# MarioPasc/MGA-YOLO

Hardware: AMD Instinct MI355X
Metric: images/s (MaskCBAM fwd+bwd step at P3/P4/P5, YOLOv8n 640x640) (higher is better)
Workload: dtype f32; 1 GPU; YOLOv8n+MGA-CBAM P3/P4/P5, 32x640x640 synthetic per GPU, fp32 (BASELINE.json configs[1]); batch_per_gpu=32, global_batch=32, parallelism=dp1, launch=hipGraph replay, 1 graph/step, handoff_kernels=True

## Files before the change

### mga_yolo_amd/_lib.py

```python
from __future__ import annotations

import ctypes as C
import os
import threading
from typing import NamedTuple

_PKG = os.path.dirname(os.path.abspath(__file__))
LIB_PATH = os.environ.get("MGACBAM_LIB") or os.path.join(_PKG, "libmgacbam.so")
ABI_VERSION = 15
MAX_LEVELS = 8
F32, F16, BF16 = 0, 1, 2
E_NULL, E_SHAPE, E_DTYPE, E_ALIGN, E_LEVELS, E_SIZE = -1, -2, -3, -4, -5, -6
E_ARG = -7
FWD_STAGES = dict(pool=1, chan=2, apply=4)
BWD_STAGES = dict(reduce1=1, convT=2, reduce2=4, wsa=8, params=16, apply=32)
BWD_FUSE = 64
FWD_SAVE_PROJ, BWD_HAVE_PROJ, PROJ_MAX_HIDDEN = 1, 1, 4
LAYOUT_NHWC = 2
FWD_ALL, BWD_PARAMS, BWD_INPUTS, BWD_ALL = 7, 31, 32, 127
BWD_FOLD = 128
FWD_FUSE = 8

_c_float_p = C.POINTER(C.c_float)

# ... 446 lines not shown
    return nbytes


def seg_ws_bytes(levels, n: int) -> int:
    return _table_size("mgaseg_ws_bytes", E_SHAPE, levels, n)


def targets_scratch_bytes(desc) -> int:
    return _table_size("mgatgt_scratch_bytes", E_ARG, C.byref(desc), zero_is_an_answer=True)


def det_ws_bytes(desc) -> int:
    return _table_size("mgadet_ws_bytes", E_ARG, C.byref(desc))


def nms_ws_bytes(desc) -> int:
    return _table_size("mganms_ws_bytes", E_ARG, C.byref(desc))


def match_ws_bytes(desc) -> int:
    return _table_size("mgamatch_ws_bytes", E_ARG, C.byref(desc))


def sync_regions(B, Cc, H, W) -> dict:
    nf = B * ((H * W + 15) // 16 + 1)
    out, o = {}, 0
    for name, n in (("gate", nf), ("status", 4), ("ca", B), ("tiles", nf), ("conv_tiles", nf), ("merged_tiles", nf),
                    ("merged_conv_tiles", nf), ("wsa_tiles", nf), ("sweeps", B * Cc)):
        out[name] = (o, n)
        o += n
    return out


def sync_len(B, Cc, H, W) -> int:
    o, n = sync_regions(B, Cc, H, W)["sweeps"]
    return o + n


def sync_slices(B, Cc, H, W) -> dict:
    return {name: slice(o, o + n) for name, (o, n) in sync_regions(B, Cc, H, W).items()}


def ctx_layout(B, Cc, H, W, hidden) -> dict:
    key = ("layout", B, Cc, H, W, hidden)
    lay = _size_cache.get(key)
    if lay is None:
        L = CtxLayout()
        check(load().mgacbam_ctx_layout(B, Cc, H, W, hidden, C.byref(L)), "mgacbam_ctx_layout")
        lay = _size_cache[key] = {n: getattr(L, n) for n in CTX_FIELDS}
    return dict(lay)
```

### mga_yolo_amd/csrc/api_fwd.hip

```cpp
#include "host.cuh"
#include "fwd.cuh"
#include "nhwc_fwd.cuh"

struct FwdSig {
  int dtype, vec, has_mask, k, proj, gvec, nhwc, weight;
  bool operator==(const FwdSig& o) const {
    return dtype == o.dtype && vec == o.vec && has_mask == o.has_mask && k == o.k && proj == o.proj && gvec == o.gvec && nhwc == o.nhwc;
  }
};
static int forward_args(const mgacbam_fwd_level_t& L, FwdArgs& A, FwdSig& sig) {
  const bool nhwc = (L.flags & MGACBAM_LAYOUT_NHWC) != 0;
  if (!L.x || !L.y || !L.ctx || (nhwc && !L.ws))
    return fail(MGACBAM_E_NULL, nhwc ? "forward (NHWC): x / y / ctx / ws is NULL" : "forward: x / y / ctx is NULL");
  if (int e = check_level("forward", L)) return e;
  const int VEC = level_vec(nhwc, L.C, L.H, L.W, L.dtype);
  const size_t need = VEC * elem_size(L.dtype);
  if (!aligned_to(L.x, need) || !aligned_to(L.y, need) || !aligned_to(L.ctx, 16) || (nhwc && !aligned_to(L.ws, 16)) ||
      (L.mask && !aligned_to(L.mask, nhwc ? 4 : 16)))
    return fail(MGACBAM_E_ALIGN, "forward%s: x/y must be %zu-byte aligned, ctx%s 16-byte, mask %d-byte", nhwc ? " (NHWC)" : "", need,
                nhwc ? " / ws" : "", nhwc ? 4 : VEC * 4);
  if (int e = check_ctx_capacity("forward", L)) return e;
  if (nhwc) if (int e = check_capacity("forward", "ws", nhwc_ws_bytes(L.B, L.C, L.H, L.W, VEC), L.ws_bytes)) return e;
  A.x = L.x; A.mask = L.mask; A.y = L.y; A.fused = 0;
  level_setup(L, A);
  A.fault = knobs().fault;
  A.n = NhwcGeo{}; A.ws = nullptr;
  sig = FwdSig{};
  sig.dtype = L.dtype; sig.vec = VEC; sig.has_mask = L.mask != nullptr; sig.k = L.p.k; sig.nhwc = nhwc;
  if (nhwc) {
    A.n = nhwc_geo(L.C, L.H, L.W, VEC);
    A.ws = static_cast<float*>(L.ws);
    const int rows = std::min((A.n.ch - 1) / L.W + 2, L.H);
    A.t.apply_rows = rows + L.p.k - 1;
    sig.weight = L.C;
    return 0;
  }
  sig.weight = L.C * A.t.chan_tx;
  sig.proj = (L.flags & MGACBAM_FWD_SAVE_PROJ) && L.mask != nullptr;
  A.g.proj_h = (sig.proj && L.p.hidden <= MGACBAM_PROJ_MAX_HIDDEN) ? L.p.hidden : 0;
  sig.gvec = VEC;
  if (L.dtype != MGACBAM_F32 && VEC == 4 && (static_cast<long long>(L.H) * L.W) % 8 == 0) {
    Tune t8 = A.t;
    gate_geometry(L.C, L.H, L.W, L.p.k, 8, t8);
    if (t8.gate_tx > 0) { sig.gvec = 8; A.t = t8; }
  }
  return 0;
}

static int launch_mlp(Group<FwdArgs>& G, hipStream_t st) {
  return launch_group("k_mlp", k_mlp, G, [](const FwdArgs& a) { return a.g.B; }, [](const FwdArgs& a) { return mlp_smem(a.g); }, st);
}

static int forward_group_nhwc(FwdArgs* lv, int n, const FwdSig& sig, int stages, hipStream_t st);
static int forward_group(FwdArgs* lv, int n, const FwdSig& sig, int stages, hipStream_t st) {
  if (sig.nhwc) return forward_group_nhwc(lv, n, sig, stages, st);
  const int pool_cpt = group_cpt(lv, n);
  for (int l = 0; l < n; ++l) lv[l].t.pool_cpt = pool_cpt;
  Group<FwdArgs> G = make_group(lv, n);

  const int gvec = sig.gvec;
  bool gate = (stages & MGACBAM_FWD_FUSE) && (stages & MGACBAM_FWD_CHAN) && (stages & MGACBAM_FWD_APPLY) && !sig.proj && gvec > 0;
  for (int l = 0; l < n && gate; ++l) gate = lv[l].t.gate_tx > 0;
  void (*gate_kernel)(GateGroup) = nullptr;
  size_t gsmem = 0;
  if (gate) {
    int span = 0;
    for (int l = 0; l < n; ++l) span = std::max(span, lv[l].t.gate_span);
    gsmem = group_smem(G, [&](const FwdArgs& a) { return gate_smem(a.g, a.t, gvec); });
    gate_kernel = with_elem_vec8(sig.dtype, gvec, [&](auto t, auto v) {
      return with_k7(sig.k, [&](auto k) { return k_gate<elem_t<decltype(t)>, v.value, k.value>; }); });
    gate = 2 * (8 * span + 1) <= resident_workgroups(gate_kernel, gsmem);
  }
  if (gate) for (int l = 0; l < n; ++l) { lv[l].fused = 1; G.lv[l].fused = 1; }

  if (stages & MGACBAM_FWD_POOL) {
    auto kernel = with_elem_vec(sig.dtype, sig.vec, [&](auto t, auto v) { return with_cpt(pool_cpt, [&](auto c) {
      return with_bool(sig.has_mask, [&](auto m) { return k_pool<elem_t<decltype(t)>, v.value, c.value, m.value>; }); }); });
    if (int e = launch_group("k_pool", kernel, G, [&](const FwdArgs& a) { return sweep_blocks(a, a.t.pool_tx, pool_cpt); }, 0, st)) return e;
  }
  if (gate) {
    GateGroup GG;
    const int tiles = fill_starts(G, lv, n, [&](const FwdArgs& a) { return xcd_grid(a.g.B, gate_tiles(a.t, a.g.H, a.g.W, gvec)); });
    GG.g = G;
    GG.nrole = 0;
    for (int l = 0; l < n; ++l) { GG.rstart[l] = GG.nrole; GG.nrole += lv[l].g.B; }
    GG.rstart[n] = GG.nrole;
    return launch("k_gate", gate_kernel, GG.nrole + tiles, kBlock, gsmem, st, GG);
  }
  if (stages & MGACBAM_FWD_CHAN) {
    bool split_mlp = false;
    for (int l = 0; l < n; ++l) split_mlp |= static_cast<long long>(lv[l].g.C) * lv[l].g.hidden >= 8192;
    if (split_mlp) if (int e = launch_mlp(G, st)) return e;
    auto kernel = with_elem_vec(sig.dtype, sig.vec, [&](auto t, auto v) { return with_bool(sig.proj, [&](auto pj) {
      return with_bool(split_mlp, [&](auto sp) { return k_chan<elem_t<decltype(t)>, v.value, pj.value, sp.value>; }); }); });
    if (int e = launch_group("k_chan", kernel, G, [&](const FwdArgs& a) { return xcd_grid(a.g.B, chan_tiles(a.t, a.g.H, a.g.W, sig.vec)); },
                             [&](const FwdArgs& a) { return chan_smem(a.g, sig.vec, sig.proj); }, st)) return e;
  }
  if (stages & MGACBAM_FWD_APPLY) {
    auto kernel = with_elem_vec(sig.dtype, sig.vec, [&](auto t, auto v) {
      return with_k(sig.k, [&](auto k) { return k_apply<elem_t<decltype(t)>, v.value, k.value>; }); });
    if (int e = launch_group("k_apply", kernel, G, [&](const FwdArgs& a) { return xcd_grid(a.g.B, chan_tiles(a.t, a.g.H, a.g.W, sig.vec)); },
                             [&](const FwdArgs& a) { return apply_smem(a.g, a.t, sig.vec); }, st)) return e;
  }
  return 0;
}

static int forward_group_nhwc(FwdArgs* lv, int n, const FwdSig& sig, int stages, hipStream_t st) {
  Group<FwdArgs> G = make_group(lv, n);
  if (stages & MGACBAM_FWD_POOL) {
    auto pool = with_elem_vec8(sig.dtype, sig.vec, [&](auto t, auto v) {
      return with_bool(sig.has_mask, [&](auto m) { return k_pool_nhwc<elem_t<decltype(t)>, v.value, m.value>; }); });
    if (int e = launch_group("k_pool_nhwc", pool, G, [](const FwdArgs& a) { return xcd_grid(a.g.B, a.n.nchunk); },
                             [](const FwdArgs& a) { return nhwc_pool_smem(a.g); }, st)) return e;
    auto fin = with_bool(sig.has_mask, [](auto m) { return k_pool_fin<m.value>; });
    if (int e = launch_group("k_pool_fin", fin, G, [](const FwdArgs& a) { return nhwc_fold_blocks(a.g); }, 0, st)) return e;
    if (int e = launch_mlp(G, st)) return e;
  }
// ... 23 lines not shown
```

### mga_yolo_amd/csrc/args.cuh

```cuda
#pragma once
#include <stddef.h>
#include <stdint.h>

namespace mgacbam {

struct Geo {
  int B, C, H, W, HW;
  int hidden, k;
  int use_sigmoid;
  float thr, eps;
  int proj_h;
};
constexpr int kProjMax = 4;
constexpr int kProjWide = 16;
constexpr int kGateR = 16;
constexpr int kSyncPx = 16;

struct CtxPtrs {
  float* S; float* use; float* den;
  float* avg; float* mx; float* mavg;
  int* valid; int* amax;
  float* h_avg; float* h_mx; float* ca;
  float* planes; int* cidx; float* sa;
  float* proj;
  int* sync;
};

struct ParamPtrs { const float* w1; const float* b1; const float* w2; const float* b2; const float* wsa; const float* beta; };

struct Tune {
  int pool_tx;
  int pool_cpt;
  int chan_tx;
  int conv_twq;
  int conv_th;
  int wsa_th;
  int apply_rows;
  int gate_rows;
  int gate_tx;
  int gate_span;
};

struct NhwcGeo {
  int cs, lcs;
  int ng;
  int ch;
  int ntile;
  int rp;
  int nchunk;
};
constexpr int kNhwcMaxChunks = 64;
constexpr int kNhwcFoldC = 64;

struct FwdArgs {
  const void* x; const float* mask; void* y;
  CtxPtrs c; ParamPtrs p; Geo g; Tune t;
  int nflag;
  int fused;
  unsigned spin_limit;
  int fault;
  long long* trace;
  NhwcGeo n;
  float* ws;
};

struct ScratchPtrs {
  float* A_part;
  float* gpre;
  float* gplanes;
  float* gwsa_part;
  float* gz;
  float* gbq;
  float* gh_avg;
  float* gh_mx;
  float* pgh;
  float* proj;
};

struct BwdArgs {
  const void* x; const float* mask; const void* gy; void* gx; float* gmask;
  float* gw1; float* gb1; float* gw2; float* gb2; float* gwsa; float* gbeta;
  CtxPtrs c; ParamPtrs p; ScratchPtrs s; Geo g; Tune t;
  int nt;
  int nconv;
// ... 32 lines not shown
```

### mga_yolo_amd/csrc/common.cuh

```cuda
#pragma once
#include <hip/hip_runtime.h>
#include <hip/hip_fp16.h>
#include <hip/hip_bf16.h>
#include <float.h>
#include <stdint.h>

#include "args.cuh"

namespace mgacbam {

constexpr int kBlock = 256;
constexpr int kSweepPF = 1;
constexpr int kWave = 64;
using bf16_t = __hip_bfloat16;

template <typename T> __device__ __forceinline__ float to_f32(T v);
template <> __device__ __forceinline__ float to_f32<float>(float v) { return v; }
template <> __device__ __forceinline__ float to_f32<__half>(__half v) { return __half2float(v); }
template <> __device__ __forceinline__ float to_f32<bf16_t>(bf16_t v) { return __bfloat162float(v); }

template <typename T> __device__ __forceinline__ T from_f32(float v);
template <> __device__ __forceinline__ float from_f32<float>(float v) { return v; }
template <> __device__ __forceinline__ __half from_f32<__half>(float v) { return __float2half_rn(v); }
template <> __device__ __forceinline__ bf16_t from_f32<bf16_t>(float v) { return __float2bfloat16(v); }
// ... 149 lines not shown
    }
    __syncthreads();
    const int waves_per_row = TX >> 6;
    if ((tid & (TX - 1)) == 0) {
#pragma unroll
      for (int n = 0; n < N; ++n) {
        for (int w = 1; w < waves_per_row; ++w) argmax_combine(v[n], idx[n], red[(wave + w) * N + n], redi[(wave + w) * N + n]);
      }
    }
  }
}

__device__ __forceinline__ float block_sum(float v, int tid, float* red) {
  v = wave_group_sum(v, kWave);
  __syncthreads();
  if ((tid & 63) == 0) red[tid >> 6] = v;
  __syncthreads();
  if (tid == 0) { v = red[0]; for (int w = 1; w < kBlock / kWave; ++w) v += red[w]; }
  return v;
}

__device__ __forceinline__ int ilog2(int v) { return 31 - __clz(v); }

__device__ __forceinline__ void bilinear_tap(float scale, int d, int n, int& i0, int& i1, float& lam) {
  const float f = fmaxf(scale * (static_cast<float>(d) + 0.5f) - 0.5f, 0.f);
  i0 = min(static_cast<int>(f), n - 1);
  i1 = i0 + (i0 < n - 1 ? 1 : 0);
  lam = f - static_cast<float>(i0);
}

__device__ __forceinline__ bool xcd_sample_part(int bid, int B, int P, int& b, int& part) {
  const int x = bid & 7, q = bid >> 3;
  const int g8 = q / P;
  part = q - g8 * P;
  b = g8 * 8 + x;
  return b < B;
}

__device__ __forceinline__ float ld_agent(const float* p) { return __hip_atomic_load(p, __ATOMIC_RELAXED, __HIP_MEMORY_SCOPE_AGENT); }
__device__ __forceinline__ int ld_agent(const int* p) { return __hip_atomic_load(p, __ATOMIC_RELAXED, __HIP_MEMORY_SCOPE_AGENT); }
__device__ __forceinline__ void st_agent(float* p, float v) { __hip_atomic_store(p, v, __ATOMIC_RELAXED, __HIP_MEMORY_SCOPE_AGENT); }
__device__ __forceinline__ void st_agent(int* p, int v) { __hip_atomic_store(p, v, __ATOMIC_RELAXED, __HIP_MEMORY_SCOPE_AGENT); }
__device__ __forceinline__ void handoff_publish(int* flag) {
  asm volatile("s_waitcnt vmcnt(0)" ::: "memory");
  __syncthreads();
  if (threadIdx.x == 0) __hip_atomic_fetch_add(flag, 1, __ATOMIC_RELAXED, __HIP_MEMORY_SCOPE_AGENT);
// ... 52 lines not shown
```

### mga_yolo_amd/csrc/fwd.cuh

```cuda
#pragma once
#include "args.cuh"
#include "common.cuh"
#include "tile.cuh"

namespace mgacbam {

constexpr float kSelLogit = 0x1.8p-24f;

template <typename T, int VEC, int CPT, bool HAS_MASK>
__device__ __forceinline__ void pool_body(const FwdArgs& A, const int bid, float* red) {
  const Geo& g = A.g;
  const int tid = threadIdx.x;
  const int TX = A.t.pool_tx, lt = ilog2(TX);
  const int tx = tid & (TX - 1), ty = tid >> lt, TY = kBlock >> lt;
  const int CPB = TY * CPT;
  const int ncg = (g.C + CPB - 1) / CPB;
  int b, cg;
  if (!xcd_sample_part(bid, g.B, ncg, b, cg)) return;
  const int c0 = cg * CPB + ty * CPT;
  const int nv = g.HW / VEC;
  TRACE_HWID(A.trace, blockIdx.x);
  TRACE_MARK(A.trace, blockIdx.x, 0);

  const T* xr[CPT];
#pragma unroll
  for (int j = 0; j < CPT; ++j) {
    const int c = min(c0 + j, g.C - 1);
    xr[j] = static_cast<const T*>(A.x) + (static_cast<size_t>(b) * g.C + c) * g.HW;
  }
  const float* mb = HAS_MASK ? A.mask + static_cast<size_t>(b) * g.HW : nullptr;
  float* splane = A.c.planes + (static_cast<size_t>(b) * 3 + 2) * g.HW;
  const bool writes_plane = (cg == 0 && ty == 0);

  float sx[CPT], sxs[CPT], vmax[CPT];
  int imax[CPT];
#pragma unroll
  for (int j = 0; j < CPT; ++j) { sx[j] = 0.f; sxs[j] = 0.f; vmax[j] = -FLT_MAX; imax[j] = 0; }
  float ssum = 0.f;

  constexpr int PF = kSweepPF;
  for (int i0 = tx; i0 < nv; i0 += TX * PF) {
    float m[PF][VEC], xv[PF][CPT][VEC];
    bool ok[PF];
#pragma unroll
    for (int p = 0; p < PF; ++p) {
      const int i = i0 + p * TX;
      ok[p] = i < nv;
      const size_t o = static_cast<size_t>(ok[p] ? i : nv - 1) * VEC;
      if (HAS_MASK) load_vec<float, VEC>(mb + o, m[p]);
#pragma unroll
      for (int j = 0; j < CPT; ++j) load_vec<T, VEC>(xr[j] + o, xv[p][j]);
    }
#pragma unroll
    for (int p = 0; p < PF; ++p) {
      if (!ok[p]) continue;
// ... 34 lines not shown
  row_argmax<CPT>(vmax, imax, TX, tid, red);

  if (tx == 0) {
    const float N = static_cast<float>(g.HW);
    const float S = sums[2 * CPT];
    const float use = (S / N >= g.thr) ? 1.f : 0.f;
    const float den = fmaxf(S, g.eps);
#pragma unroll
    for (int j = 0; j < CPT; ++j) {
      const int c = c0 + j;
      if (c < g.C) {
        const size_t o = static_cast<size_t>(b) * g.C + c;
        const float gap = sums[j] / N;
        float avg, mavg, mxo;
        int valid;
        if (HAS_MASK) {
          mavg = sums[CPT + j] / den;
          avg = mavg * use + gap * (1.f - use);
          valid = isclosef_(vmax[j], -FLT_MAX) ? 0 : 1;
          mxo = valid ? vmax[j] : gap;
        } else {
          mavg = gap; avg = gap; valid = 1; mxo = vmax[j];
        }
        A.c.avg[o] = avg; A.c.mavg[o] = mavg; A.c.mx[o] = mxo;
        A.c.valid[o] = valid; A.c.amax[o] = imax[j];
      }
    }
    if (cg == 0 && ty == 0) {
      A.c.S[b] = HAS_MASK ? S : 0.f;
      A.c.use[b] = HAS_MASK ? use : 0.f;
      A.c.den[b] = HAS_MASK ? den : 1.f;
    }
  }
#ifdef MGACBAM_TRACE
  TRACE_MARK(A.trace, blockIdx.x, 8);
  asm volatile("s_waitcnt vmcnt(0)" ::: "memory");
  __syncthreads();
  TRACE_MARK(A.trace, blockIdx.x, 10);
#endif
}

template <typename T, int VEC, int CPT, bool HAS_MASK>
__global__ __launch_bounds__(kBlock) void k_pool(const Group<FwdArgs> G) {
  __shared__ float red[64];
  int local;
  const int l = find_level(G, blockIdx.x, local);
  pool_body<T, VEC, CPT, HAS_MASK>(G.lv[l], local, red);
}

__device__ __forceinline__ void mlp_gate_to_lds(const FwdArgs& A, const int b, const bool publish,
                                                float* s_in, float* s_h, float* s_ca) {
  const Geo& g = A.g;
  const int tid = threadIdx.x, C = g.C, h = g.hidden;
  const int wave = tid >> 6, lane = tid & 63;
  float* s_avg = s_in;
  float* s_mx = s_in + C;
  for (int c = tid; c < C; c += kBlock) {
    s_avg[c] = A.c.avg[static_cast<size_t>(b) * C + c];
    s_mx[c] = A.c.mx[static_cast<size_t>(b) * C + c];
  }
  __syncthreads();
  for (int j = wave; j < h; j += kBlock / kWave) {
    const float* w = A.p.w1 + static_cast<size_t>(j) * C;
    float da = 0.f, dm = 0.f;
    for (int c = lane; c < C; c += kWave) { const float wv = w[c]; da += wv * s_avg[c]; dm += wv * s_mx[c]; }
    da = wave_group_sum(da, kWave);
    dm = wave_group_sum(dm, kWave);
    if (lane == 0) {
      const float bj = A.p.b1[j];
      const float ha = fmaxf(da + bj, 0.f), hm = fmaxf(dm + bj, 0.f);
// ... 281 lines not shown
  const int nv = g.HW / VEC;
  const int ntile = (nv + TX - 1) / TX;
  int b, tile;
  if (!xcd_sample_part(bid, g.B, ntile, b, tile)) return;
  const int i = tile * TX + tx;
  const bool active = i < nv;
  const int ii = active ? i : nv - 1;
  const size_t base = static_cast<size_t>(b) * g.C * g.HW + static_cast<size_t>(ii) * VEC;
  const T* xp = static_cast<const T*>(A.x) + base;
  T* yp = static_cast<T*>(A.y) + base;

  const int gid = blockIdx.x;
  TRACE_HWID(A.trace, gid);
  TRACE_MARK(A.trace, gid, 0);
  Pack<T, VEC> xr[R];
#pragma unroll
  for (int j = 0; j < R; ++j)
    xr[j] = *reinterpret_cast<const Pack<T, VEC>*>(xp + static_cast<size_t>(min(ty + j * TY, g.C - 1)) * g.HW);
  int* flags = A.c.sync + static_cast<size_t>(b) * A.nflag;
  const int gen = static_cast<int>(static_cast<unsigned>(ld_agent(flags + tile)) + 1u);

  float* s_ca = smem;
  float* work = s_ca + ((g.C + 3) & ~3);
  bool bad;
  {
    int* caflag = A.c.sync + static_cast<size_t>(g.B) * A.nflag + 4;
    bad = handoff_wait(caflag, b, b, gen, caflag - 4, A.spin_limit);
    const float* cab = A.c.ca + static_cast<size_t>(b) * g.C;
    TRACE_MARK(A.trace, gid, 1);
    for (int c = tid; c < g.C; c += kBlock) s_ca[c] = ld_agent(cab + c);
    __syncthreads();
  }
  TRACE_MARK(A.trace, gid, 2);

  float vmax[VEC], vsum[VEC];
  int vidx[VEC];
#pragma unroll
  for (int e = 0; e < VEC; ++e) { vmax[e] = -INFINITY; vsum[e] = 0.f; vidx[e] = ty; }
#pragma unroll
  for (int j = 0; j < R; ++j) {
    const int c = ty + j * TY;
    if (c < g.C) {
      const float cac = s_ca[c];
#pragma unroll
      for (int e = 0; e < VEC; ++e) {
        const float uu = to_f32<T>(xr[j].v[e]) * cac;
        vsum[e] += uu;
        if (uu > vmax[e]) { vmax[e] = uu; vidx[e] = c; }
      }
    }
  }
  TRACE_MARK(A.trace, gid, 3);
  {
// ... 112 lines not shown
#pragma unroll
  for (int j = 0; j < R; ++j) {
    const int c = ty + j * TY;
    if (c < g.C) {
      const float cac = s_ca[c];
      float yv[VEC];
#pragma unroll
      for (int e = 0; e < VEC; ++e) {
        const float xe = to_f32<T>(xr[j].v[e]);
        const float u = xe * cac;
        yv[e] = xe + a * (u * sav[e] - xe);
      }
      if (active) store_vec<T, VEC>(yp + static_cast<size_t>(c) * g.HW, yv);
    }
  }
#ifdef MGACBAM_TRACE
  TRACE_MARK(A.trace, gid, 9);
  asm volatile("s_waitcnt vmcnt(0)" ::: "memory");
  __syncthreads();
  TRACE_MARK(A.trace, gid, 10);
#endif
}

constexpr int kMlpW1 = 8;
constexpr int kMlpW2 = 8;
__device__ __forceinline__ bool mlp_stream_ok(const Geo& g) { return (g.C & 3) == 0 && (g.hidden & 3) == 0 && g.C <= 8 * 4 * kWave; }

template <int CVL>
__device__ __forceinline__ void mlp_hidden(const FwdArgs& A, const int b, float* s_avg, float* s_mx, float* s_h) {
  constexpr int UP = kMlpW1 / CVL;
  const Geo& g = A.g;
  const int tid = threadIdx.x, C = g.C, h = g.hidden, CV = C >> 2;
  const int wave = tid >> 6, lane = tid & 63;
  const float4* w1v = reinterpret_cast<const float4*>(A.p.w1);
  const int nunit = h > wave ? (h - wave + 3) >> 2 : 0;
  const int npass = (((h + 3) >> 2) + UP - 1) / UP;
  for (int p = 0; p < npass; ++p) {
    float4 wr[UP][CVL];
#pragma unroll
    for (int uu = 0; uu < UP; ++uu) {
      const int u = p * UP + uu, j = wave + 4 * u;
#pragma unroll
      for (int i = 0; i < CVL; ++i) {
        const int cv = lane + kWave * i;
        wr[uu][i] = (u < nunit && cv < CV) ? w1v[static_cast<size_t>(j) * CV + cv] : float4{0.f, 0.f, 0.f, 0.f};
      }
    }
    if (p == 0) {
      for (int c = tid; c < C; c += kBlock) {
        s_avg[c] = A.c.avg[static_cast<size_t>(b) * C + c];
        s_mx[c] = A.c.mx[static_cast<size_t>(b) * C + c];
      }
      __syncthreads();
    }
#pragma unroll
    for (int uu = 0; uu < UP; ++uu) {
      const int u = p * UP + uu;
      if (u < nunit) {
        float da = 0.f, dm = 0.f;
#pragma unroll
        for (int i = 0; i < CVL; ++i) {
          const int cv = lane + kWave * i;
          if (cv < CV) {
            const float4 w = wr[uu][i];
            const float4 a4 = *reinterpret_cast<const float4*>(s_avg + 4 * cv), m4 = *reinterpret_cast<const float4*>(s_mx + 4 * cv);
            da += w.x * a4.x + w.y * a4.y + w.z * a4.z + w.w * a4.w;
            dm += w.x * m4.x + w.y * m4.y + w.z * m4.z + w.w * m4.w;
          }
        }
        da = wave_group_sum(da, kWave);
        dm = wave_group_sum(dm, kWave);
        if (lane == 0) {
          const int j = wave + 4 * u;
          const float bj = A.p.b1[j];
          const float ha = fmaxf(da + bj, 0.f), hm = fmaxf(dm + bj, 0.f);
          s_h[j] = ha; s_h[h + j] = hm;
          A.c.h_avg[static_cast<size_t>(b) * h + j] = ha;
          A.c.h_mx[static_cast<size_t>(b) * h + j] = hm;
        }
      }
    }
  }
}

template <bool AGENT>
__device__ __forceinline__ void mlp_stream(const FwdArgs& A, const int b, float* smem) {
  const Geo& g = A.g;
  const int tid = threadIdx.x, C = g.C, h = g.hidden;
  float* s_avg = smem;
  float* s_mx = smem + C;
  float* s_h = smem + 2 * C;
  const int cvl = ((C >> 2) + kWave - 1) / kWave;
  if (cvl <= 1) mlp_hidden<1>(A, b, s_avg, s_mx, s_h);
  else if (cvl <= 2) mlp_hidden<2>(A, b, s_avg, s_mx, s_h);
  else if (cvl <= 4) mlp_hidden<4>(A, b, s_avg, s_mx, s_h);
  else mlp_hidden<8>(A, b, s_avg, s_mx, s_h);
  const int HV = h >> 2;
  const float4* w2v = reinterpret_cast<const float4*>(A.p.w2);
  float4 wr[kMlpW2];
  {
    const int c = min(tid, C - 1);
#pragma unroll
    for (int q = 0; q < kMlpW2; ++q) wr[q] = q < HV ? w2v[static_cast<size_t>(c) * HV + q] : float4{0.f, 0.f, 0.f, 0.f};
  }
  __syncthreads();
  for (int c = tid; c < C; c += kBlock) {
    float za = 0.f, zm = 0.f;
    for (int v0 = 0; v0 < HV; v0 += kMlpW2) {
      if (c != tid || v0 != 0) {
#pragma unroll
        for (int q = 0; q < kMlpW2; ++q) wr[q] = v0 + q < HV ? w2v[static_cast<size_t>(c) * HV + v0 + q] : float4{0.f, 0.f, 0.f, 0.f};
      }
#pragma unroll
      for (int q = 0; q < kMlpW2; ++q) {
        if (v0 + q < HV) {
          const float* ha = s_h + 4 * (v0 + q);
          const float* hm = ha + h;
          za += wr[q].x * ha[0]; zm += wr[q].x * hm[0];
          za += wr[q].y * ha[1]; zm += wr[q].y * hm[1];
          za += wr[q].z * ha[2]; zm += wr[q].z * hm[2];
          za += wr[q].w * ha[3]; zm += wr[q].w * hm[3];
        }
      }
    }
    const float bc = A.p.b2[c];
    const float ca = sigmoidf_((za + bc) + (zm + bc));
    if (AGENT) st_agent(A.c.ca + static_cast<size_t>(b) * C + c, ca);
    else A.c.ca[static_cast<size_t>(b) * C + c] = ca;
  }
}

__device__ __forceinline__ void gate_role(const FwdArgs& A, const int b, float* smem) {
  const Geo& g = A.g;
  const int tid = threadIdx.x, C = g.C, h = g.hidden;
  int* caflag = A.c.sync + static_cast<size_t>(g.B) * A.nflag + 4 + b;
  TRACE_MARK(A.trace, blockIdx.x, 0);
  if (mlp_stream_ok(g)) {
// ... 58 lines not shown
```

### mga_yolo_amd/csrc/host.cuh

```cuda
#pragma once
#include "../../include/mgacbam.h"

#include <hip/hip_runtime.h>
#include <stdarg.h>
#include <stdio.h>
#include <stdlib.h>
#include <string.h>

#include <algorithm>
#include <atomic>
#include <map>
#include <mutex>
#include <type_traits>
#include <utility>

#include "args.cuh"
#include "common.cuh"

using namespace mgacbam;

inline thread_local char g_err[512] = "";
static int fail(int code, const char* fmt, ...) {
  va_list ap;
  va_start(ap, fmt);
// ... 7 lines not shown
  void* p[] = {const_cast<void*>(static_cast<const void*>(&args))...};
  const hipError_t e = hipLaunchKernel(reinterpret_cast<const void*>(kernel), dim3(static_cast<unsigned>(grid)), dim3(block), p, smem, st);
  if (e != hipSuccess) return fail(static_cast<int>(e), "%s: %s", what, hipGetErrorString(e));
  return 0;
}

static int check_shape(int B, int C, int H, int W, int hidden, int k) {
  if (B < 1 || C < 1 || H < 1 || W < 1 || hidden < 1 || hidden > 4096 || C > 65536)
    return fail(MGACBAM_E_SHAPE, "bad shape B=%d C=%d H=%d W=%d hidden=%d", B, C, H, W, hidden);
  if (static_cast<long long>(H) * W > (1ll << 30) || static_cast<long long>(B) * C * H * W > (1ll << 40))
    return fail(MGACBAM_E_SHAPE, "tensor too large B=%d C=%d H=%d W=%d", B, C, H, W);
  if (k < 1 || k > 15 || (k & 1) == 0) return fail(MGACBAM_E_SHAPE, "spatial kernel k=%d must be odd and in 1..15", k);
  return 0;
}

struct SyncLayout {
  size_t nflag;
  size_t gate;
  size_t status;
  size_t ca;
  size_t bflag, cflag;
  size_t mbflag, mcflag;
  size_t wflag, sflag;
  size_t len;
};
static SyncLayout sync_layout(int B, int C, size_t HW) {
  SyncLayout S;
  S.nflag = (HW + kSyncPx - 1) / kSyncPx + 1;
  const size_t per = static_cast<size_t>(B) * S.nflag;
  S.gate = 0; S.status = per; S.ca = S.status + 4; S.bflag = S.ca + B;
  S.cflag = S.bflag + per; S.mbflag = S.cflag + per; S.mcflag = S.mbflag + per; S.wflag = S.mcflag + per; S.sflag = S.wflag + per;
  S.len = S.sflag + static_cast<size_t>(B) * C;
  return S;
}

struct Carver {
  size_t total = 0;
  size_t take(size_t n_elems) { const size_t off = total; total = align16(total + n_elems * 4); return off; }
};
template <typename T = float>
static T* at(const void* base, size_t off) { return reinterpret_cast<T*>(static_cast<char*>(const_cast<void*>(base)) + off); }

static void ctx_layout(int B, int C, int H, int W, int hidden, mgacbam_ctx_layout_t* L) {
  const size_t HW = static_cast<size_t>(H) * W, BC = static_cast<size_t>(B) * C;
  Carver cv;
  L->S = cv.take(B); L->use = cv.take(B); L->den = cv.take(B);
  L->avg = cv.take(BC); L->mx = cv.take(BC); L->mavg = cv.take(BC);
  L->valid = cv.take(BC); L->amax = cv.take(BC);
  L->h_avg = cv.take(static_cast<size_t>(B) * hidden); L->h_mx = cv.take(static_cast<size_t>(B) * hidden);
  L->ca = cv.take(BC);
  L->planes = cv.take(static_cast<size_t>(B) * 3 * HW);
  L->cidx = cv.take(static_cast<size_t>(B) * HW);
  L->sa = cv.take(static_cast<size_t>(B) * HW);
  L->proj = cv.take(hidden <= MGACBAM_PROJ_MAX_HIDDEN ? static_cast<size_t>(B) * hidden * HW : 0);
  const SyncLayout S = sync_layout(B, C, HW);
// ... 1 lines not shown
  L->status = L->sync + static_cast<int64_t>(4 * S.status);
  L->total = static_cast<int64_t>(cv.total);
}

static CtxPtrs ctx_ptrs(void* p, int B, int C, int H, int W, int hidden) {
  mgacbam_ctx_layout_t L;
  ctx_layout(B, C, H, W, hidden, &L);
  return CtxPtrs{at(p, L.S), at(p, L.use), at(p, L.den), at(p, L.avg), at(p, L.mx), at(p, L.mavg), at<int>(p, L.valid), at<int>(p, L.amax),
                 at(p, L.h_avg), at(p, L.h_mx), at(p, L.ca), at(p, L.planes), at<int>(p, L.cidx), at(p, L.sa), at(p, L.proj), at<int>(p, L.sync)};
}

static int pow2_floor(int v) { int p = 1; while (p * 2 <= v) p *= 2; return p; }
static int pow2_ceil(int v) { int p = 1; while (p < v) p *= 2; return p; }
static int env_int(const char* name, int dflt) {
  const char* s = getenv(name);
  return (s && *s) ? atoi(s) : dflt;
}
struct Knobs {
  int bwd_merge;
  int gate_narrow;
  int pool_tx, pool_cpt, chan_tx;
  int resident_wgs;
  int fault;
  unsigned spin_limit;
  long long* trace;
};
static Knobs read_knobs() {
  Knobs k;
  k.bwd_merge = env_int("MGACBAM_BWD_MERGE", 1);
  k.gate_narrow = env_int("MGACBAM_GATE_NARROW", 0);
  k.pool_tx = env_int("MGACBAM_POOL_TX", 0); k.pool_cpt = env_int("MGACBAM_POOL_CPT", 0); k.chan_tx = env_int("MGACBAM_CHAN_TX", 0);
  k.resident_wgs = env_int("MGACBAM_RESIDENT_WGS", 0); k.fault = env_int("MGACBAM_FAULT", 0);
  const int sl = env_int("MGACBAM_SPIN_LIMIT", 0);
  k.spin_limit = sl > 0 ? static_cast<unsigned>(sl) : (1u << 20);
  const char* tp = getenv("MGACBAM_TRACE_PTR");
  k.trace = (tp && *tp) ? reinterpret_cast<long long*>(strtoull(tp, nullptr, 0)) : nullptr;
  return k;
}
inline std::mutex g_knob_mu;
inline Knobs g_knobs;
inline std::atomic<bool> g_knobs_ready{false};
static Knobs knobs() {
  if (!g_knobs_ready.load(std::memory_order_acquire)) {
    std::lock_guard<std::mutex> lk(g_knob_mu);
    if (!g_knobs_ready.load(std::memory_order_relaxed)) { g_knobs = read_knobs(); g_knobs_ready.store(true, std::memory_order_release); }
  }
  return g_knobs;
}

static int device_cus() {
  static std::mutex mu;
  static int cus[64] = {0};
  int dev = 0;
  if (hipGetDevice(&dev) != hipSuccess || dev < 0 || dev >= 64) return 0;
  std::lock_guard<std::mutex> lk(mu);
// ... 21 lines not shown
    int n = 0;
    if (hipOccupancyMaxActiveBlocksPerMultiprocessor(&n, kernel, kBlock, smem) != hipSuccess) n = 0;
    per_cu = n;
    std::lock_guard<std::mutex> lk(mu);
    cache[key] = per_cu;
  }
  return per_cu * device_cus();
}
static bool is_pow2_in(int v, int lo, int hi) { return v >= lo && v <= hi && (v & (v - 1)) == 0; }

static int vec_of(int H, int W) { return (static_cast<long long>(H) * W) % 4 == 0 ? 4 : 1; }

static void gate_geometry(int C, int H, int W, int k, int VEC, Tune& t) {
  t.gate_tx = 0; t.gate_rows = 0; t.gate_span = 0;
  const int gty = pow2_ceil((C + kGateR - 1) / kGateR);
  if (gty > kBlock) return;
  const int gtx = kBlock / gty, TP = gtx * VEC;
  int grows = (TP - 1) / W + 2;
  if (grows > H) grows = H;
  grows += k - 1;
  const int span = ((k / 2) * W + TP - 1) / TP + 1;
  const size_t lds = (3 * static_cast<size_t>(grows) * (W + k - 1) + TP + 3 * k * k + 3 * C + 64) * sizeof(float);
  if (TP >= kSyncPx && (TP >= W || knobs().gate_narrow) && lds <= 48 * 1024) { t.gate_tx = gtx; t.gate_rows = grows; t.gate_span = span; }
}

static Tune choose_tune(int B, int C, int H, int W, int k) {
  const int HW = H * W, VEC = vec_of(H, W), nv = HW / VEC;
  const Knobs kn = knobs();
  Tune t;
  int tx = pow2_floor(nv / 4 > 0 ? nv / 4 : 1);
  if (tx > 256) tx = 256;
  int cpt = 4;
  while (cpt > 1 && static_cast<long long>(B) * ((C + (256 / tx) * cpt - 1) / ((256 / tx) * cpt)) < 1024) cpt /= 2;
  t.pool_tx = tx; t.pool_cpt = cpt;
  int ctx = pow2_ceil(nv) < 64 ? pow2_ceil(nv) : 64;
  constexpr int kChanMinTx = 16;
  while (ctx > kChanMinTx && static_cast<long long>(B) * ((nv + ctx - 1) / ctx) < 768) ctx /= 2;
  while (ctx < 64 && (256 / ctx) * 4 > C) ctx *= 2;
  t.chan_tx = ctx;
  const int ntx = (W + 127) / 128;
  const int tw = (((W + ntx - 1) / ntx) + 3) / 4 * 4;
  t.conv_twq = tw / 4;
  int th = 256 / t.conv_twq;
  if (th > H) th = H;
  if (th > 64) th = 64;
  const int cap = 24 * 256 / (4 * (tw + k - 1)) - (k - 1);
// ... 202 lines not shown
static int params_blocks(const Geo& g) { return g.hidden + (g.C + kBlock - 1) / kBlock + (3 * g.k * g.k + 3) / 4 + 1; }
static size_t chan_smem(const Geo& g, int vec, bool proj) {
  return (3 * static_cast<size_t>(g.C) + 2 * g.hidden + (proj ? static_cast<size_t>(g.C) * kProjMax : 0) + 4 * kBlock * vec) * sizeof(float);
}
static size_t apply_smem(const Geo& g, const Tune& t, int vec) {
  return (((3 * g.k * g.k + 3) & ~3) + 3 * static_cast<size_t>(t.apply_rows) * (g.W + g.k - 1) + t.chan_tx * vec + g.C) * sizeof(float);
}
static size_t gate_smem(const Geo& g, const Tune& t, int vec) {
  const size_t head = (g.C + 3) & ~3;
  const size_t role = 3 * static_cast<size_t>(g.C) + 2 * g.hidden;
  const size_t conv = ((3 * g.k * g.k + 3) & ~3) + 3 * static_cast<size_t>(t.gate_rows) * (g.W + g.k - 1) + static_cast<size_t>(t.gate_tx) * vec;
  return std::max(role, head + std::max(conv, static_cast<size_t>(3) * kBlock * vec)) * sizeof(float);
}
static int gate_tiles(const Tune& t, int H, int W, int vec) {
  const int nv = H * W / vec;
  return (nv + t.gate_tx - 1) / t.gate_tx;
}
static size_t bwd_apply_smem(const Geo& g, int vec) { return (5 * static_cast<size_t>(g.C) + 2 * g.hidden + kBlock * vec) * sizeof(float); }
static size_t reduce1_smem(const Geo& g, int vec, int proj) {
  if (!proj) return (3 * static_cast<size_t>(g.C) + kBlock * vec) * sizeof(float);
  if (proj == 2) return (((3 * static_cast<size_t>(g.C) + 3) & ~static_cast<size_t>(3)) + 3 * 16 * kWave) * sizeof(float);
  return (((3 * static_cast<size_t>(g.C) + 3) & ~static_cast<size_t>(3)) + static_cast<size_t>(g.C) * kProjMax + 4 * kBlock * vec) * sizeof(float);
}
static size_t mlp_smem(const Geo& g) { return (3 * static_cast<size_t>(g.C) + 2 * g.hidden) * sizeof(float); }
static size_t nhwc_pool_smem(const Geo& g) { return 4 * static_cast<size_t>(g.C) * sizeof(float); }
static size_t nhwc_chan_smem(const Geo& g) { return static_cast<size_t>(g.C) * sizeof(float); }
static size_t nhwc_apply_smem(const Geo& g, const Tune& t, const NhwcGeo& n) {
  return (((3 * g.k * g.k + 3) & ~3) + 3 * static_cast<size_t>(t.apply_rows) * (g.W + g.k - 1) + n.ch + g.C) * sizeof(float);
}
static size_t nhwc_reduce1_smem(const Geo& g, int vec) {
  return (3 * ((static_cast<size_t>(g.C) + 3) & ~static_cast<size_t>(3)) + 2 * kBlock * vec) * sizeof(float);
}
static size_t nhwc_reduce2_smem(const Geo& g) { return static_cast<size_t>(g.C) * sizeof(float); }
static size_t nhwc_bwd_apply_smem(const Geo& g) { return (5 * static_cast<size_t>(g.C) + 2 * g.hidden) * sizeof(float); }

template <typename Args, typename Fn>
static int fill_starts(Group<Args>& G, const Args* lv, int n, Fn blocks_of) {
  int tot = 0;
  for (int l = 0; l < n; ++l) { G.start[l] = tot; tot += blocks_of(lv[l]); }
  G.start[n] = tot;
  return tot;
}
template <typename Args>
static Group<Args> make_group(const Args* lv, int n) {
  Group<Args> G;
  G.n = n;
// ... 50 lines not shown
```

Baseline: 169,200 images/s.

## Compute channel-attention MLP in the last-arriving pool block per image

Adds a per-image arrival counter so that the last pool workgroup to finish an image runs the channel MLP, using a streaming variant with fewer weight registers, and writes the channel attention. The fused gate kernel then skips its role workgroups for those levels and reads the attention directly instead of spin-waiting on a handoff flag. It is enabled by default for large levels and is meant to take the MLP off the gate kernel's critical path. In exchange it adds an atomic tail to the pool kernel, grows the sync buffer, and bumps the ca flag without a wait.

```diff
diff --git a/mga_yolo_amd/_lib.py b/mga_yolo_amd/_lib.py
--- a/mga_yolo_amd/_lib.py
+++ b/mga_yolo_amd/_lib.py
@@ -492,18 +492,21 @@
     return _table_size("mgamatch_ws_bytes", E_ARG, C.byref(desc))
 
 
+ARRIVE_STRIDE = 64
+
+
 def sync_regions(B, Cc, H, W) -> dict:
     nf = B * ((H * W + 15) // 16 + 1)
     out, o = {}, 0
     for name, n in (("gate", nf), ("status", 4), ("ca", B), ("tiles", nf), ("conv_tiles", nf), ("merged_tiles", nf),
-                    ("merged_conv_tiles", nf), ("wsa_tiles", nf), ("sweeps", B * Cc)):
+                    ("merged_conv_tiles", nf), ("wsa_tiles", nf), ("sweeps", B * Cc), ("arrive", B * ARRIVE_STRIDE)):
         out[name] = (o, n)
         o += n
     return out
 
 
 def sync_len(B, Cc, H, W) -> int:
-    o, n = sync_regions(B, Cc, H, W)["sweeps"]
+    o, n = sync_regions(B, Cc, H, W)["arrive"]
     return o + n
 
 
diff --git a/mga_yolo_amd/csrc/api_fwd.hip b/mga_yolo_amd/csrc/api_fwd.hip
--- a/mga_yolo_amd/csrc/api_fwd.hip
+++ b/mga_yolo_amd/csrc/api_fwd.hip
@@ -24,6 +24,8 @@
   A.x = L.x; A.mask = L.mask; A.y = L.y; A.fused = 0;
   level_setup(L, A);
   A.fault = knobs().fault;
+  A.pool_mlp = 0;
+  A.arrive0 = static_cast<int>(sync_layout(L.B, L.C, static_cast<size_t>(L.H) * L.W).arrive);
   A.n = NhwcGeo{}; A.ws = nullptr;
   sig = FwdSig{};
   sig.dtype = L.dtype; sig.vec = VEC; sig.has_mask = L.mask != nullptr; sig.k = L.p.k; sig.nhwc = nhwc;
@@ -44,6 +46,7 @@
     gate_geometry(L.C, L.H, L.W, L.p.k, 8, t8);
     if (t8.gate_tx > 0) { sig.gvec = 8; A.t = t8; }
   }
+  A.pool_mlp = pool_forms_ca(A.g, A.t, false, L.dtype);
   return 0;
 }
 
@@ -73,17 +76,22 @@
   }
   if (gate) for (int l = 0; l < n; ++l) { lv[l].fused = 1; G.lv[l].fused = 1; }
 
+  bool any_pool_mlp = false, all_pool_mlp = true;
+  for (int l = 0; l < n; ++l) { any_pool_mlp |= lv[l].pool_mlp != 0; all_pool_mlp &= lv[l].pool_mlp != 0; }
+
   if (stages & MGACBAM_FWD_POOL) {
     auto kernel = with_elem_vec(sig.dtype, sig.vec, [&](auto t, auto v) { return with_cpt(pool_cpt, [&](auto c) {
-      return with_bool(sig.has_mask, [&](auto m) { return k_pool<elem_t<decltype(t)>, v.value, c.value, m.value>; }); }); });
-    if (int e = launch_group("k_pool", kernel, G, [&](const FwdArgs& a) { return sweep_blocks(a, a.t.pool_tx, pool_cpt); }, 0, st)) return e;
+      return with_bool(sig.has_mask, [&](auto m) { return with_bool(any_pool_mlp, [&](auto ml) {
+        return k_pool<elem_t<decltype(t)>, v.value, c.value, m.value, ml.value>; }); }); }); });
+    if (int e = launch_group("k_pool", kernel, G, [&](const FwdArgs& a) { return sweep_blocks(a, a.t.pool_tx, pool_cpt); },
+                             [](const FwdArgs& a) { return a.pool_mlp ? pool_mlp_smem(a.g) : size_t(0); }, st)) return e;
   }
   if (gate) {
     GateGroup GG;
     const int tiles = fill_starts(G, lv, n, [&](const FwdArgs& a) { return xcd_grid(a.g.B, gate_tiles(a.t, a.g.H, a.g.W, gvec)); });
     GG.g = G;
     GG.nrole = 0;
-    for (int l = 0; l < n; ++l) { GG.rstart[l] = GG.nrole; GG.nrole += lv[l].g.B; }
+    for (int l = 0; l < n; ++l) { GG.rstart[l] = GG.nrole; GG.nrole += lv[l].pool_mlp ? 0 : lv[l].g.B; }
     GG.rstart[n] = GG.nrole;
     return launch("k_gate", gate_kernel, GG.nrole + tiles, kBlock, gsmem, st, GG);
   }
@@ -91,8 +99,9 @@
     bool split_mlp = false;
     for (int l = 0; l < n; ++l) split_mlp |= static_cast<long long>(lv[l].g.C) * lv[l].g.hidden >= 8192;
     if (split_mlp) if (int e = launch_mlp(G, st)) return e;
+    const bool have_ca = split_mlp || all_pool_mlp;
     auto kernel = with_elem_vec(sig.dtype, sig.vec, [&](auto t, auto v) { return with_bool(sig.proj, [&](auto pj) {
-      return with_bool(split_mlp, [&](auto sp) { return k_chan<elem_t<decltype(t)>, v.value, pj.value, sp.value>; }); }); });
+      return with_bool(have_ca, [&](auto sp) { return k_chan<elem_t<decltype(t)>, v.value, pj.value, sp.value>; }); }); });
     if (int e = launch_group("k_chan", kernel, G, [&](const FwdArgs& a) { return xcd_grid(a.g.B, chan_tiles(a.t, a.g.H, a.g.W, sig.vec)); },
                              [&](const FwdArgs& a) { return chan_smem(a.g, sig.vec, sig.proj); }, st)) return e;
   }
diff --git a/mga_yolo_amd/csrc/args.cuh b/mga_yolo_amd/csrc/args.cuh
--- a/mga_yolo_amd/csrc/args.cuh
+++ b/mga_yolo_amd/csrc/args.cuh
@@ -15,6 +15,7 @@
 constexpr int kProjWide = 16;
 constexpr int kGateR = 16;
 constexpr int kSyncPx = 16;
+constexpr int kArriveStride = 64;
 
 struct CtxPtrs {
   float* S; float* use; float* den;
@@ -60,6 +61,8 @@
   unsigned spin_limit;
   int fault;
   long long* trace;
+  int pool_mlp;
+  int arrive0;
   NhwcGeo n;
   float* ws;
 };
diff --git a/mga_yolo_amd/csrc/common.cuh b/mga_yolo_amd/csrc/common.cuh
--- a/mga_yolo_amd/csrc/common.cuh
+++ b/mga_yolo_amd/csrc/common.cuh
@@ -195,6 +195,8 @@
 
 __device__ __forceinline__ int ilog2(int v) { return 31 - __clz(v); }
 
+__host__ __device__ __forceinline__ bool mlp_stream_ok(const Geo& g) { return (g.C & 3) == 0 && (g.hidden & 3) == 0 && g.C <= 8 * 4 * kWave; }
+
 __device__ __forceinline__ void bilinear_tap(float scale, int d, int n, int& i0, int& i1, float& lam) {
   const float f = fmaxf(scale * (static_cast<float>(d) + 0.5f) - 0.5f, 0.f);
   i0 = min(static_cast<int>(f), n - 1);
diff --git a/mga_yolo_amd/csrc/fwd.cuh b/mga_yolo_amd/csrc/fwd.cuh
--- a/mga_yolo_amd/csrc/fwd.cuh
+++ b/mga_yolo_amd/csrc/fwd.cuh
@@ -7,8 +7,14 @@
 
 constexpr float kSelLogit = 0x1.8p-24f;
 
-template <typename T, int VEC, int CPT, bool HAS_MASK>
-__device__ __forceinline__ void pool_body(const FwdArgs& A, const int bid, float* red) {
+constexpr int kMlpW1 = 8;
+constexpr int kMlpW2 = 8;
+constexpr int kPoolMlpW = 2;
+template <bool AGENT, bool LDA = false, int NW1 = kMlpW1, int NW2 = kMlpW2>
+__device__ __forceinline__ void mlp_stream(const FwdArgs& A, const int b, float* smem);
+
+template <typename T, int VEC, int CPT, bool HAS_MASK, bool MLP>
+__device__ __forceinline__ void pool_body(const FwdArgs& A, const int bid, float* red, float* smem) {
   const Geo& g = A.g;
   const int tid = threadIdx.x;
   const int TX = A.t.pool_tx, lt = ilog2(TX);
@@ -31,6 +37,7 @@
   const float* mb = HAS_MASK ? A.mask + static_cast<size_t>(b) * g.HW : nullptr;
   float* splane = A.c.planes + (static_cast<size_t>(b) * 3 + 2) * g.HW;
   const bool writes_plane = (cg == 0 && ty == 0);
+  const bool tail = MLP && A.pool_mlp;
 
   float sx[CPT], sxs[CPT], vmax[CPT];
   int imax[CPT];
@@ -111,7 +118,9 @@
         } else {
           mavg = gap; avg = gap; valid = 1; mxo = vmax[j];
         }
-        A.c.avg[o] = avg; A.c.mavg[o] = mavg; A.c.mx[o] = mxo;
+        if (tail) { st_agent(A.c.avg + o, avg); st_agent(A.c.mx + o, mxo); }
+        else { A.c.avg[o] = avg; A.c.mx[o] = mxo; }
+        A.c.mavg[o] = mavg;
         A.c.valid[o] = valid; A.c.amax[o] = imax[j];
       }
     }
@@ -127,14 +136,31 @@
   __syncthreads();
   TRACE_MARK(A.trace, blockIdx.x, 10);
 #endif
-}
-
-template <typename T, int VEC, int CPT, bool HAS_MASK>
+  if constexpr (MLP) {
+    if (!tail) return;
+    int* arrive = A.c.sync + A.arrive0 + static_cast<size_t>(b) * kArriveStride;
+    int* s_last = reinterpret_cast<int*>(smem);
+    asm volatile("s_waitcnt vmcnt(0)" ::: "memory");
+    __syncthreads();
+    if (tid == 0) {
+      const int before = __hip_atomic_fetch_add(arrive, 1, __ATOMIC_RELAXED, __HIP_MEMORY_SCOPE_AGENT);
+      if (before == ncg - 1) st_agent(arrive, 0);
+      *s_last = before == ncg - 1;
+    }
+    __syncthreads();
+    if (!*s_last) return;
+    mlp_stream<false, true, kPoolMlpW, kPoolMlpW>(A, b, smem + 4);
+    TRACE_MARK(A.trace, blockIdx.x, 11);
+  }
+}
+
+template <typename T, int VEC, int CPT, bool HAS_MASK, bool MLP = false>
 __global__ __launch_bounds__(kBlock) void k_pool(const Group<FwdArgs> G) {
   __shared__ float red[64];
+  extern __shared__ __align__(16) float pool_smem[];
   int local;
   const int l = find_level(G, blockIdx.x, local);
-  pool_body<T, VEC, CPT, HAS_MASK>(G.lv[l], local, red);
+  pool_body<T, VEC, CPT, HAS_MASK, MLP>(G.lv[l], local, red, pool_smem);
 }
 
 __device__ __forceinline__ void mlp_gate_to_lds(const FwdArgs& A, const int b, const bool publish,
@@ -462,13 +488,20 @@
 
   float* s_ca = smem;
   float* work = s_ca + ((g.C + 3) & ~3);
-  bool bad;
+  bool bad = false;
   {
-    int* caflag = A.c.sync + static_cast<size_t>(g.B) * A.nflag + 4;
-    bad = handoff_wait(caflag, b, b, gen, caflag - 4, A.spin_limit);
     const float* cab = A.c.ca + static_cast<size_t>(b) * g.C;
-    TRACE_MARK(A.trace, gid, 1);
-    for (int c = tid; c < g.C; c += kBlock) s_ca[c] = ld_agent(cab + c);
+    if (A.pool_mlp) {
+      TRACE_MARK(A.trace, gid, 1);
+      for (int c = tid; c < g.C; c += kBlock) s_ca[c] = cab[c];
+      if (tile == 0 && tid == 0)
+        __hip_atomic_fetch_add(A.c.sync + static_cast<size_t>(g.B) * A.nflag + 4 + b, 1, __ATOMIC_RELAXED, __HIP_MEMORY_SCOPE_AGENT);
+    } else {
+      int* caflag = A.c.sync + static_cast<size_t>(g.B) * A.nflag + 4;
+      bad = handoff_wait(caflag, b, b, gen, caflag - 4, A.spin_limit);
+      TRACE_MARK(A.trace, gid, 1);
+      for (int c = tid; c < g.C; c += kBlock) s_ca[c] = ld_agent(cab + c);
+    }
     __syncthreads();
   }
   TRACE_MARK(A.trace, gid, 2);
@@ -627,13 +660,11 @@
 #endif
 }
 
-constexpr int kMlpW1 = 8;
-constexpr int kMlpW2 = 8;
-__device__ __forceinline__ bool mlp_stream_ok(const Geo& g) { return (g.C & 3) == 0 && (g.hidden & 3) == 0 && g.C <= 8 * 4 * kWave; }
-
-template <int CVL>
+
+template <int CVL, bool LDA, int NW1>
 __device__ __forceinline__ void mlp_hidden(const FwdArgs& A, const int b, float* s_avg, float* s_mx, float* s_h) {
-  constexpr int UP = kMlpW1 / CVL;
+  constexpr int UP = NW1 > CVL ? NW1 / CVL : 1;
+  constexpr int CH = NW1 < CVL ? NW1 : CVL;
   const Geo& g = A.g;
   const int tid = threadIdx.x, C = g.C, h = g.hidden, CV = C >> 2;
   const int wave = tid >> 6, lane = tid & 63;
@@ -641,44 +672,55 @@
   const int nunit = h > wave ? (h - wave + 3) >> 2 : 0;
   const int npass = (((h + 3) >> 2) + UP - 1) / UP;
   for (int p = 0; p < npass; ++p) {
-    float4 wr[UP][CVL];
-#pragma unroll
-    for (int uu = 0; uu < UP; ++uu) {
-      const int u = p * UP + uu, j = wave + 4 * u;
-#pragma unroll
-      for (int i = 0; i < CVL; ++i) {
-        const int cv = lane + kWave * i;
-        wr[uu][i] = (u < nunit && cv < CV) ? w1v[static_cast<size_t>(j) * CV + cv] : float4{0.f, 0.f, 0.f, 0.f};
-      }
-    }
-    if (p == 0) {
-      for (int c = tid; c < C; c += kBlock) {
-        s_avg[c] = A.c.avg[static_cast<size_t>(b) * C + c];
-        s_mx[c] = A.c.mx[static_cast<size_t>(b) * C + c];
-      }
-      __syncthreads();
+    float da[UP], dm[UP];
+#pragma unroll
+    for (int uu = 0; uu < UP; ++uu) { da[uu] = 0.f; dm[uu] = 0.f; }
+#pragma unroll 1
+    for (int i0 = 0; i0 < CVL; i0 += CH) {
+      float4 wr[UP][CH];
+#pragma unroll
+      for (int uu = 0; uu < UP; ++uu) {
+        const int u = p * UP + uu, j = wave + 4 * u;
+#pragma unroll
+        for (int i = 0; i < CH; ++i) {
+          const int cv = lane + kWave * (i0 + i);
+          wr[uu][i] = (u < nunit && cv < CV) ? w1v[static_cast<size_t>(j) * CV + cv] : float4{0.f, 0.f, 0.f, 0.f};
+        }
+      }
+      if (p == 0 && i0 == 0) {
+        for (int c = tid; c < C; c += kBlock) {
+          const float* pa = A.c.avg + static_cast<size_t>(b) * C + c;
+          const float* pm = A.c.mx + static_cast<size_t>(b) * C + c;
+          s_avg[c] = LDA ? ld_agent(pa) : *pa;
+          s_mx[c] = LDA ? ld_agent(pm) : *pm;
+        }
+        __syncthreads();
+      }
+#pragma unroll
+      for (int uu = 0; uu < UP; ++uu) {
+        if (p * UP + uu < nunit) {
+#pragma unroll
+          for (int i = 0; i < CH; ++i) {
+            const int cv = lane + kWave * (i0 + i);
+            if (cv < CV) {
+              const float4 w = wr[uu][i];
+              const float4 a4 = *reinterpret_cast<const float4*>(s_avg + 4 * cv), m4 = *reinterpret_cast<const float4*>(s_mx + 4 * cv);
+              da[uu] += w.x * a4.x + w.y * a4.y + w.z * a4.z + w.w * a4.w;
+              dm[uu] += w.x * m4.x + w.y * m4.y + w.z * m4.z + w.w * m4.w;
+            }
+          }
+        }
+      }
     }
 #pragma unroll
     for (int uu = 0; uu < UP; ++uu) {
       const int u = p * UP + uu;
       if (u < nunit) {
-        float da = 0.f, dm = 0.f;
-#pragma unroll
-        for (int i = 0; i < CVL; ++i) {
-          const int cv = lane + kWave * i;
-          if (cv < CV) {
-            const float4 w = wr[uu][i];
-            const float4 a4 = *reinterpret_cast<const float4*>(s_avg + 4 * cv), m4 = *reinterpret_cast<const float4*>(s_mx + 4 * cv);
-            da += w.x * a4.x + w.y * a4.y + w.z * a4.z + w.w * a4.w;
-            dm += w.x * m4.x + w.y * m4.y + w.z * m4.z + w.w * m4.w;
-          }
-        }
-        da = wave_group_sum(da, kWave);
-        dm = wave_group_sum(dm, kWave);
+        const float sa = wave_group_sum(da[uu], kWave), sm = wave_group_sum(dm[uu], kWave);
         if (lane == 0) {
           const int j = wave + 4 * u;
           const float bj = A.p.b1[j];
-          const float ha = fmaxf(da + bj, 0.f), hm = fmaxf(dm + bj, 0.f);
+          const float ha = fmaxf(sa + bj, 0.f), hm = fmaxf(sm + bj, 0.f);
           s_h[j] = ha; s_h[h + j] = hm;
           A.c.h_avg[static_cast<size_t>(b) * h + j] = ha;
           A.c.h_mx[static_cast<size_t>(b) * h + j] = hm;
@@ -688,7 +730,7 @@
   }
 }
 
-template <bool AGENT>
+template <bool AGENT, bool LDA, int NW1, int NW2>
 __device__ __forceinline__ void mlp_stream(const FwdArgs& A, const int b, float* smem) {
   const Geo& g = A.g;
   const int tid = threadIdx.x, C = g.C, h = g.hidden;
@@ -696,28 +738,28 @@
   float* s_mx = smem + C;
   float* s_h = smem + 2 * C;
   const int cvl = ((C >> 2) + kWave - 1) / kWave;
-  if (cvl <= 1) mlp_hidden<1>(A, b, s_avg, s_mx, s_h);
-  else if (cvl <= 2) mlp_hidden<2>(A, b, s_avg, s_mx, s_h);
-  else if (cvl <= 4) mlp_hidden<4>(A, b, s_avg, s_mx, s_h);
-  else mlp_hidden<8>(A, b, s_avg, s_mx, s_h);
+  if (cvl <= 1) mlp_hidden<1, LDA, NW1>(A, b, s_avg, s_mx, s_h);
+  else if (cvl <= 2) mlp_hidden<2, LDA, NW1>(A, b, s_avg, s_mx, s_h);
+  else if (cvl <= 4) mlp_hidden<4, LDA, NW1>(A, b, s_avg, s_mx, s_h);
+  else mlp_hidden<8, LDA, NW1>(A, b, s_avg, s_mx, s_h);
   const int HV = h >> 2;
   const float4* w2v = reinterpret_cast<const float4*>(A.p.w2);
-  float4 wr[kMlpW2];
+  float4 wr[NW2];
   {
     const int c = min(tid, C - 1);
 #pragma unroll
-    for (int q = 0; q < kMlpW2; ++q) wr[q] = q < HV ? w2v[static_cast<size_t>(c) * HV + q] : float4{0.f, 0.f, 0.f, 0.f};
+    for (int q = 0; q < NW2; ++q) wr[q] = q < HV ? w2v[static_cast<size_t>(c) * HV + q] : float4{0.f, 0.f, 0.f, 0.f};
   }
   __syncthreads();
   for (int c = tid; c < C; c += kBlock) {
     float za = 0.f, zm = 0.f;
-    for (int v0 = 0; v0 < HV; v0 += kMlpW2) {
+    for (int v0 = 0; v0 < HV; v0 += NW2) {
       if (c != tid || v0 != 0) {
 #pragma unroll
-        for (int q = 0; q < kMlpW2; ++q) wr[q] = v0 + q < HV ? w2v[static_cast<size_t>(c) * HV + v0 + q] : float4{0.f, 0.f, 0.f, 0.f};
-      }
-#pragma unroll
-      for (int q = 0; q < kMlpW2; ++q) {
+        for (int q = 0; q < NW2; ++q) wr[q] = v0 + q < HV ? w2v[static_cast<size_t>(c) * HV + v0 + q] : float4{0.f, 0.f, 0.f, 0.f};
+      }
+#pragma unroll
+      for (int q = 0; q < NW2; ++q) {
         if (v0 + q < HV) {
           const float* ha = s_h + 4 * (v0 + q);
           const float* hm = ha + h;
diff --git a/mga_yolo_amd/csrc/host.cuh b/mga_yolo_amd/csrc/host.cuh
--- a/mga_yolo_amd/csrc/host.cuh
+++ b/mga_yolo_amd/csrc/host.cuh
@@ -53,6 +53,7 @@
   size_t bflag, cflag;
   size_t mbflag, mcflag;
   size_t wflag, sflag;
+  size_t arrive;
   size_t len;
 };
 static SyncLayout sync_layout(int B, int C, size_t HW) {
@@ -61,7 +62,8 @@
   const size_t per = static_cast<size_t>(B) * S.nflag;
   S.gate = 0; S.status = per; S.ca = S.status + 4; S.bflag = S.ca + B;
   S.cflag = S.bflag + per; S.mbflag = S.cflag + per; S.mcflag = S.mbflag + per; S.wflag = S.mcflag + per; S.sflag = S.wflag + per;
-  S.len = S.sflag + static_cast<size_t>(B) * C;
+  S.arrive = S.sflag + static_cast<size_t>(B) * C;
+  S.len = S.arrive + static_cast<size_t>(B) * kArriveStride;
   return S;
 }
 
@@ -109,6 +111,7 @@
   int pool_tx, pool_cpt, chan_tx;
   int resident_wgs;
   int fault;
+  int pool_mlp;
   unsigned spin_limit;
   long long* trace;
 };
@@ -118,6 +121,7 @@
   k.gate_narrow = env_int("MGACBAM_GATE_NARROW", 0);
   k.pool_tx = env_int("MGACBAM_POOL_TX", 0); k.pool_cpt = env_int("MGACBAM_POOL_CPT", 0); k.chan_tx = env_int("MGACBAM_CHAN_TX", 0);
   k.resident_wgs = env_int("MGACBAM_RESIDENT_WGS", 0); k.fault = env_int("MGACBAM_FAULT", 0);
+  k.pool_mlp = env_int("MGACBAM_POOL_MLP", 1);
   const int sl = env_int("MGACBAM_SPIN_LIMIT", 0);
   k.spin_limit = sl > 0 ? static_cast<unsigned>(sl) : (1u << 20);
   const char* tp = getenv("MGACBAM_TRACE_PTR");
@@ -185,6 +189,13 @@
   const int span = ((k / 2) * W + TP - 1) / TP + 1;
   const size_t lds = (3 * static_cast<size_t>(grows) * (W + k - 1) + TP + 3 * k * k + 3 * C + 64) * sizeof(float);
   if (TP >= kSyncPx && (TP >= W || knobs().gate_narrow) && lds <= 48 * 1024) { t.gate_tx = gtx; t.gate_rows = grows; t.gate_span = span; }
+}
+
+static bool pool_forms_ca(const Geo& g, const Tune& t, bool nhwc, int dtype) {
+  const Knobs kn = knobs();
+  if (nhwc || kn.fault || kn.pool_mlp == 0) return false;
+  if (!mlp_stream_ok(g) || static_cast<long long>(g.C) * g.hidden >= 8192 || t.gate_tx <= 0) return false;
+  return kn.pool_mlp == 2 || static_cast<size_t>(g.C) * g.HW * (dtype == MGACBAM_F32 ? 4 : 2) >= (size_t(1) << 20);
 }
 
 static Tune choose_tune(int B, int C, int H, int W, int k) {
@@ -433,6 +444,7 @@
   if (proj == 2) return (((3 * static_cast<size_t>(g.C) + 3) & ~static_cast<size_t>(3)) + 3 * 16 * kWave) * sizeof(float);
   return (((3 * static_cast<size_t>(g.C) + 3) & ~static_cast<size_t>(3)) + static_cast<size_t>(g.C) * kProjMax + 4 * kBlock * vec) * sizeof(float);
 }
+static size_t pool_mlp_smem(const Geo& g) { return (4 + 2 * static_cast<size_t>(g.C) + 2 * g.hidden) * sizeof(float); }
 static size_t mlp_smem(const Geo& g) { return (3 * static_cast<size_t>(g.C) + 2 * g.hidden) * sizeof(float); }
 static size_t nhwc_pool_smem(const Geo& g) { return 4 * static_cast<size_t>(g.C) * sizeof(float); }
 static size_t nhwc_chan_smem(const Geo& g) { return static_cast<size_t>(g.C) * sizeof(float); }
```

Result: faster. 172,900 images/s (median of 6 runs) (+2.2%).
